# martin-velas/SLAM_plus_plus

Measured on AMD Instinct MI355X. Metric: Lambda solve GFLOP/s (algorithmic factor+solve flops / wall-clock), 100k-pose SE(3), higher is better.
Workload: dtype f64; 1 GPU; C3: synthetic 100000-pose SE(3) chain + loop closures, 6x6 blocks, 201998 upper blocks, n=600000; numeric factor + 2 substitutions per step (symbolic analysis cached, inputs resident in HBM); parallelism=1 GPU

## Files before the change

slam_plus_plus_amd/csrc/preload.h:

```cpp
#pragma once
#include <hip/hip_runtime.h>

#define SLAMPP_PRELOAD_UNIT(unit) \
	namespace slampp { \
	__global__ void preload_##unit##_kernel() {} \
	void preload_##unit(hipStream_t stream) { hipLaunchKernelGGL(preload_##unit##_kernel, dim3(1), dim3(1), 0, stream); } \
	}

namespace slampp {

void preload_simt_kernel(hipStream_t stream);
void preload_panel_kernel(hipStream_t stream);
void preload_sparse_kernels(hipStream_t stream);
void preload_subtree_kernel(hipStream_t stream);
void preload_dense_tiles(hipStream_t stream);
void preload_dense_chol(hipStream_t stream);
void preload_schur(hipStream_t stream);
void preload_schur_tiles(hipStream_t stream);

inline void preload_device_code(hipStream_t stream)
{
	preload_simt_kernel(stream);
	preload_panel_kernel(stream);
	preload_sparse_kernels(stream);
	preload_subtree_kernel(stream);
	preload_dense_tiles(stream);
	preload_dense_chol(stream);
	preload_schur(stream);
	preload_schur_tiles(stream);
}

}
```

slam_plus_plus_amd/csrc/simt_kernel.hip:

```cpp
#include <hip/hip_runtime.h>
#include "sparse_kernels.h"

#include <algorithm>
#include <cstdio>

namespace slampp {

__device__ __forceinline__ double simt_rsqrt(double x)
{
	double y = __builtin_amdgcn_rsq(x);
	const double h = 0.5 * x;
	y = y * (1.5 - h * y * y);
	y = y * (1.5 - h * y * y);
	return y;
}

template <int D>
__device__ __forceinline__ void load_column(const double *__restrict__ p, double (&v)[D])
{
	if(D % 2 == 0) {
		const double2 *p2 = reinterpret_cast<const double2*>(p);
		#pragma unroll
		for(int i = 0; i < D / 2; ++ i) {
			const double2 t = p2[i];
			v[2 * i] = t.x;
			v[2 * i + 1] = t.y;
		}
	} else {
		#pragma unroll
		for(int i = 0; i < D; ++ i)
			v[i] = p[i];
	}
}

template <int D>
__device__ __forceinline__ void load_block(const double *__restrict__ p, double (&v)[D][D])
{
	if(D % 2 == 0) {
		const double2 *p2 = reinterpret_cast<const double2*>(p);
		#pragma unroll
		for(int i = 0; i < D * D / 2; ++ i) {
			const double2 t = p2[i];
			v[(2 * i) / D][(2 * i) % D] = t.x;
			v[(2 * i + 1) / D][(2 * i + 1) % D] = t.y;
		}
	} else {
		#pragma unroll
		for(int i = 0; i < D * D; ++ i)
			v[i / D][i % D] = p[i];
	}
}

template <int D>
__device__ __forceinline__ void load_lower(const double *__restrict__ p, double (&v)[D][D])
{
	#pragma unroll
	for(int q = 0; q < D; ++ q) {
		if(D % 2 == 0) {
			#pragma unroll
			for(int r = q & ~1; r < D; r += 2) {
				const double2 t = *reinterpret_cast<const double2*>(p + r + q * D);
				v[q][r] = t.x;
				v[q][r + 1] = t.y;
			}
		} else {
			#pragma unroll
			for(int r = q; r < D; ++ r)
				v[q][r] = p[r + q * D];
		}
	}
}

template <int D>
__device__ __forceinline__ void store_block(double *p, const double (&m)[D][D])
{
	if(D % 2 == 0) {
		double2 *p2 = reinterpret_cast<double2*>(p);
		#pragma unroll
		for(int q = 0; q < D; ++ q) {
			#pragma unroll
			for(int r = 0; r < D; r += 2)
				p2[(r + q * D) / 2] = double2{m[r][q], m[r + 1][q]};
		}
	} else {
		#pragma unroll
		for(int q = 0; q < D; ++ q) {
			#pragma unroll
			for(int r = 0; r < D; ++ r)
				p[r + q * D] = m[r][q];
		}
	}
}

template <int D>
__device__ __forceinline__ void load_half_rows(const double *__restrict__ p, int r0, double (&v)[D][D / 2])
{
	#pragma unroll
	for(int c = 0; c < D; ++ c) {
		#pragma unroll
		for(int i = 0; i < D / 2; ++ i)
			v[c][i] = p[r0 + i + c * D];
	}
}

__device__ __forceinline__ int pc_next_column(const int32_t *P, int pc, int nb, int nr)
{
	pc += 2 * nr;
	for(int kb = 1; kb < nb; ++ kb)
		pc += 1 + 2 * P[pc];
	return pc;
}

template <int D, int W, int LPT, bool b_linv>
__global__ void __launch_bounds__(64)
factor_simt_kernel(const TSimtChunk *__restrict__ chunks, const int32_t *__restrict__ prog, const long long *__restrict__ tab,
	const double *__restrict__ A, double *L, double *Linv, const double *__restrict__ b, double *w, int *p_flag,
	long long *p_timing, TBatch t_batch)
{	{ const int64_t n_member = blockIdx.y; A += n_member * t_batch.a; L += n_member * t_batch.l; Linv = Linv? Linv + n_member * t_batch.linv : Linv; b += n_member * t_batch.b; w += n_member * t_batch.w; p_flag += n_member; }

	enum { DD = D * D };
	extern __shared__ long long s_tab[];
	const TSimtChunk ch = chunks[blockIdx.x];
	{
		const int n_entries = (4 * prog[ch.prog_off] + prog[ch.prog_off + 1] + prog[ch.prog_off + 2] + prog[ch.prog_off + 3]) * W;
		for(int i = threadIdx.x; i < n_entries; i += 64)
			s_tab[i] = tab[ch.tab_off + i];
		__syncthreads();
	}
	if(int(threadIdx.x) >= W * LPT)
		return;
	const int n_half = (LPT == 2)? int(threadIdx.x) & 1 : 0;
	enum { DH = (LPT == 2)? D / 2 : D };
	const int r0 = n_half * DH;
	long long *p_tm = 0;
	int n_tm = 0;
	if(p_timing && blockIdx.x == gridDim.x / 2 && threadIdx.x == 0) {
		const unsigned long long n_tm_record = atomicAdd((unsigned long long*)p_timing, 1ull);
		p_tm = (n_tm_record < 4096)? p_timing + 1 + 32 * n_tm_record : 0;
		if(p_tm)
			p_tm[n_tm ++] = wall_clock64();
	}
#define SIMT_TICK() do { if(p_tm && n_tm < 32) p_tm[n_tm ++] = wall_clock64(); } while(0)
	const int32_t *P = prog + ch.prog_off;
	const long long *T = s_tab + threadIdx.x / LPT;
// ... 187 lines not shown
				}
			}
			double *p_out = L + l_base + kb * DD;
			#pragma unroll
			for(int q = 0; q < D; ++ q) {
				double out[DH];
				#pragma unroll
				for(int i = 0; i < DH; ++ i) {
					double sum = 0;
					#pragma unroll
					for(int t = 0; t <= q; ++ t)
						sum += acc[i][t] * x[q][t];
					out[i] = sum;
				}
				if(DH % 2 == 0 && D % 2 == 0) {
					#pragma unroll
					for(int i = 0; i < DH; i += 2)
						*reinterpret_cast<double2*>(p_out + r0 + i + q * D) = double2{out[i], out[i + 1]};
				} else {
					#pragma unroll
					for(int i = 0; i < DH; ++ i)
						p_out[r0 + i + q * D] = out[i];
				}
			}
			SIMT_TICK();
		}
		blk0 += nb;
	}
	if(b_bad || f_touched == 1.2345e301)
		atomicOr(p_flag, 1);
}

bool launch_factor_simt(const TSimtChunk *chunks, int n_chunks, int n_width, int n_lds_bytes, const int32_t *prog, const int64_t *tab, int n_dim,
	const double *A, double *L, double *Linv, const double *b, double *w, int *p_flag, hipStream_t stream, long long *p_timing, const TBatch &t_batch)
{
	if(n_chunks <= 0)
		return true;
	const long long *t = reinterpret_cast<const long long*>(tab);
#define SIMT_LAUNCH(D_, W_, LPT_) do { if(Linv) hipLaunchKernelGGL((factor_simt_kernel<D_, W_, LPT_, true>), dim3(n_chunks, t_batch.n), dim3(64), n_lds_bytes, stream, chunks, prog, t, \
	A, L, Linv, b, w, p_flag, p_timing, t_batch); else hipLaunchKernelGGL((factor_simt_kernel<D_, W_, LPT_, false>), dim3(n_chunks, t_batch.n), dim3(64), n_lds_bytes, stream, chunks, prog, t, \
	A, L, Linv, b, w, p_flag, p_timing, t_batch); } while(0)
#define SIMT_WIDTHS(D_) do { if(n_width == 16) { if(b_pairs && D_ % 2 == 0) SIMT_LAUNCH(D_, 16, (D_ % 2 == 0)? 2 : 1); else SIMT_LAUNCH(D_, 16, 1); } \
	else if(n_width == 32) { if(b_pairs && D_ % 2 == 0) SIMT_LAUNCH(D_, 32, (D_ % 2 == 0)? 2 : 1); else SIMT_LAUNCH(D_, 32, 1); } \
	else SIMT_LAUNCH(D_, 64, 1); } while(0)
	const int n_pairs_env = dev_knob("SLAMPP_HIP_DEV_SIMT_PAIRS", -1);
	const bool b_pairs = (n_pairs_env >= 0)? n_pairs_env != 0 : n_chunks <= 2048;
	switch(n_dim) {
	case 3:
		SIMT_WIDTHS(3);
		return true;
	case 6:
		SIMT_WIDTHS(6);
		return true;
	case 7:
		SIMT_WIDTHS(7);
		return true;
	default:
		return false;
	}
#undef SIMT_WIDTHS
#undef SIMT_LAUNCH
}

template <int D, int W>
__global__ void __launch_bounds__(64)
backward_simt_kernel(const TSimtChunk *__restrict__ chunks, const int32_t *__restrict__ prog, const long long *__restrict__ tab,
	const double *__restrict__ L, double *w, double *x_out, TBatch t_batch)
{	{ const int64_t n_member = blockIdx.y; L += n_member * t_batch.l; w += n_member * t_batch.w; x_out += n_member * t_batch.b; }

	enum { DD = D * D };
	extern __shared__ long long s_tab[];
	const TSimtChunk ch = chunks[blockIdx.x];
	const int32_t *P = prog + ch.prog_off;
	const int n_cols = P[0], n_below = P[1];
	{
		const int n_entries = (3 * n_cols + n_below) * W;
		for(int i = threadIdx.x; i < n_entries; i += 64)
			s_tab[i] = tab[ch.tab_off + i];
		__syncthreads();
// ... 421 lines not shown
```

slam_plus_plus_amd/csrc/solver.h:

```cpp
#pragma once
#include <hip/hip_runtime.h>
#include <chrono>
#include <cstdint>
#include <new>
#include <stdexcept>
#include <string>
#include <vector>
#include <thread>
#include <memory>
#include <mutex>

#include "../../include/slampp_hip.h"
#include "plan.h"
#include "host_pool.h"
#include "sparse_records.h"
#include <utility>
#include "sparse_kernels.h"
#include "dense_chol.h"

namespace slampp {

struct CDeviceError : public std::runtime_error {
	explicit CDeviceError(const std::string &s) :std::runtime_error(s) {}
};
// ... 122 lines not shown
	void Refine_Structure();
	bool b_schur_fallback = false;
	int n_staging_ahead = 0;
	int n_schur_fallback_option = 1;
	slampp::Plan plan;
	slampp::SparseLaunchLists lists;
	slampp::TDevPlan dplan;
	slampp::CDevArray<slampp::TColDesc> d_cols;
	slampp::CDevArray<slampp::TBlkDesc> d_blks;
	slampp::CDevArray<slampp::TRowEnt> d_rents;
	slampp::CDevArray<longlong2> d_pairs;
	slampp::CDevArray<int64_t> d_task_ptr, d_task_pkg;
	slampp::CDevArray<longlong2> d_pkg;
	slampp::CDevArray<long long> d_timing;
	slampp::CDevArray<slampp::TSimtChunk> d_simt_chunks;
	slampp::CDevArray<int32_t> d_simt_prog, d_simt_rest;
	int n_panel = -1;
	int n_panel_rows = -1;
	slampp::CDevArray<longlong2> d_panel_pkg;
	slampp::CDevArray<int64_t> d_panel_off, d_panel_out_off;
	slampp::CDevArray<double> d_handup;
	int n_panel_handup = 1;
	slampp::CDevArray<int32_t> d_panel_rest;
	int n_panel_backward = -1;
	size_t n_lds_limit = 0;
	slampp::CDevArray<longlong2> d_bwd_rec;
	slampp::CDevArray<int64_t> d_bwd_off;
	slampp::CDevArray<slampp::TUpdSlot> d_panel_upd_slots;
	slampp::CDevArray<slampp::TUpdEnt> d_panel_upd_ents;
	slampp::CDevArray<int64_t> d_simt_tab;
	slampp::CDevArray<slampp::TSimtChunk> d_simt_bwd_chunks;
	slampp::CDevArray<int32_t> d_simt_bwd_prog;
	slampp::CDevArray<int64_t> d_simt_bwd_tab;
	std::vector<int32_t> simt_bwd_ahead_waves;
	bool b_leaf_linv_wanted = false, b_leaf_linv_valid = true;
	slampp::TBatch t_batch = slampp::t_No_Batch();
	slampp::CDevArray<double> d_batch_L, d_batch_Linv, d_batch_w, d_batch_handup;
	slampp::CDevArray<int> d_batch_flag;
	int n_batch_owner_member = -1;
	int *p_host_batch_flag = 0;
	int n_batch_pending = 0;
	int n_simt_backward = -1;
	void Ensure_Leaf_Inverses();
	int n_simt = -1;
	int n_wide_min_tasks = 8192;
	int n_simt_width = 32;
	int n_simt_stages = 1;
	void Upload_Simt(const slampp::SparseRecords &r_rec);
	void Report_Simt_Backward(const slampp::SparseRecords &r_rec) const;
	slampp::CDevArray<slampp::TDenseBlk> d_dense_blks;
	slampp::CDevArray<int64_t> d_dense_blk_loff;
	slampp::CDevArray<double> d_dense, d_dense_invdiag, d_dense_z, d_dense_x;
	slampp::CDevArray<int32_t> d_dense_gaps;
	int n_dense_gaps;
	slampp::CDevArray<uint8_t> d_dense_unit;
	slampp::CDevArray<longlong2> d_dense_dst;
	slampp::CTileSchedule dense_tiles;
	bool b_dense_tiles;
	bool b_dense_clean;
	int n_dense_top_tiles;
	int n_dense_blks, n_dense_cols, n_dense_dim, n_dense_pad;
	slampp::CDevArray<double> d_A, d_rhs, d_L, d_Linv, d_w, d_cov;
	slampp::CSparseInverse *p_sinv = 0;
	bool b_sinv_tried = false;
	slampp::CCovariance *p_cov = 0;
	slampp::CDevArray<double> d_Z;
	slampp::CDevArray<double> d_Zd, d_Zd_work;
	slampp::CDevArray<int64_t> d_diag_zoff;
	slampp::CDevArray<int32_t> d_diag_dim;
	slampp::CDevArray<int64_t> d_diag_out_off;
	slampp::CDevArray<int64_t> d_damp_off;
	bool b_damp_valid = false;
	bool Require_Damping_Offsets();
	slampp::CDevArray<double> d_lm_reduce;
	slampp::CDevArray<int64_t> d_state_cumsum;
	bool b_state_cumsum_valid = false;
	slampp::CDevArray<int> d_flag;
	int *p_flag_shared = 0;
	int *p_host_flag;

	double *p_pin_values = 0, *p_pin_rhs = 0;
	size_t n_pin_values = 0, n_pin_rhs = 0;
// ... 128 lines not shown
```

slam_plus_plus_amd/csrc/sparse_enqueue.hip:

```cpp
#include <execinfo.h>
#include <signal.h>
#include <unistd.h>
#include <pthread.h>
#include "solver.h"
#include "sparse_inverse.h"

#include <algorithm>
#include <atomic>
#include <chrono>
#include <cstdio>
#include <cstdlib>
#include <cstring>
#include <map>
#include <thread>
#include <mutex>
#include <condition_variable>
#include <functional>
#include <sys/mman.h>

using namespace slampp;

void slampp_hip_solver::Enqueue_Sparse(const double *p_values_dev, double *p_rhs_dev, bool b_factor, bool b_factor_only)
{
	const Plan &P = plan;
// ... 20 lines not shown
		b_panel_fused = b_panel_fused || lists.b_any_hand_up;
		auto Launch_Panels = [&](int s, bool b_bottom) {
			const int n_panels = lists.panel_ptr[s + 1] - lists.panel_ptr[s];
			const bool b_rode = lists.panel_ride[s] != 0;
			if(!b_rode)
				launch_panel_update(P.max_dim, d_panel_upd_slots.p() + lists.panel_upd_ptr[s], lists.panel_upd_ptr[s + 1] - lists.panel_upd_ptr[s],
					d_panel_upd_ents.p(), p_values_dev, d_L.p(), p_rhs_dev, d_w.p(), stream, t_batch);
			const int n_next = (s + 1 < n_stages && lists.panel_ride[s + 1] == 1)? lists.panel_upd_ptr[s + 2] - lists.panel_upd_ptr[s + 1] : 0;
			if(!launch_factor_panel(P.max_dim, b_panel_fused, (n_panel_rows < 0)? P.max_dim >= 6 : n_panel_rows != 0, lists.panel_cfg[s], d_panel_pkg.p(), d_panel_off.p() + lists.panel_ptr[s],
				d_panel_out_off.p() + lists.panel_ptr[s], n_panels,
				d_panel_upd_slots.p() + ((n_next > 0)? lists.panel_upd_ptr[s + 1] : 0), n_next, d_panel_upd_ents.p(), p_values_dev, p_rhs_dev,
				d_L.p(), d_Linv.p(), d_w.p(), d_handup.p(), p_flag, stream, dplan.p_timing, t_batch))
				throw CDeviceError("panel launch refused: block size or LDS request outside what the analysis planned for");
			if(lists.panel_rest_ptr[s + 1] > lists.panel_rest_ptr[s]) {
				TDevPlan t_rest = dplan;
				t_rest.task_map = d_panel_rest.p();
				launch_factor_stage(t_rest, p_values_dev, d_L.p(), d_Linv.p(), p_rhs_dev, d_w.p(), lists.panel_rest_ptr[s],
					lists.panel_rest_ptr[s + 1] - lists.panel_rest_ptr[s], b_bottom, p_flag, stream, t_batch);
			}
		};
		for(int s = 0; s < n_stages; ++ s) {
			if(s == 0)
				Phase_Begin("factor_leaves");
			else if(s == 1 && (b_profile >= 2 || n_wide_end <= 1))
				Phase_Begin((s < n_wide_end)? "factor_wide" : "factor_upper");
			else if(s == 1)
				Phase_Begin("factor_rest");
			else if(s == n_wide_end && b_profile >= 2)
				Phase_Begin("factor_upper");
			if(b_simt && s + 1 < int(lists.simt_chunk_ptr.size())) {
				const int n_chunks = lists.simt_chunk_ptr[s + 1] - lists.simt_chunk_ptr[s], n_rest = lists.simt_rest_ptr[s + 1] - lists.simt_rest_ptr[s];
				const bool b_store_linv = b_leaf_linv_wanted || !b_simt_backward_wanted;
				launch_factor_simt(d_simt_chunks.p() + lists.simt_chunk_ptr[s], n_chunks, n_simt_width, lists.simt_lds_bytes[s], d_simt_prog.p(), d_simt_tab.p(), P.max_dim,
					p_values_dev, d_L.p(), b_store_linv? d_Linv.p() : 0, p_rhs_dev, d_w.p(), p_flag, stream, dplan.p_timing, t_batch);
				b_leaf_linv_valid = b_leaf_linv_valid && b_store_linv;
				if(n_rest > 0) {
					TDevPlan t_rest = dplan;
					t_rest.task_map = d_simt_rest.p();
					launch_factor_stage(t_rest, p_values_dev, d_L.p(), d_Linv.p(), p_rhs_dev, d_w.p(), lists.simt_rest_ptr[s], n_rest,
						true, p_flag, stream, t_batch);
				}
			} else if(s == 0 && !lists.panel_ptr.empty() && lists.panel_ptr[1] > lists.panel_ptr[0]) {
				Launch_Panels(s, true);
			} else if(s > 0 && s < lists.n_bottom_stages && dplan.task_pkg)
				launch_factor_wide(dplan, p_values_dev, d_L.p(), d_Linv.p(), p_rhs_dev, d_w.p(), P.stage_ptr[s],
					P.stage_ptr[s + 1] - P.stage_ptr[s], p_flag, stream, t_batch);
			else if(s >= lists.n_bottom_stages && !lists.panel_ptr.empty()) {
				Launch_Panels(s, false);
			} else
			launch_factor_stage(dplan, p_values_dev, d_L.p(), d_Linv.p(), p_rhs_dev, d_w.p(), P.stage_ptr[s],
				P.stage_ptr[s + 1] - P.stage_ptr[s], s < lists.n_bottom_stages, p_flag, stream, t_batch);
			if(s == 0 || (s == n_wide_end - 1 && b_profile >= 2) || s == n_stages - 1)
				Phase_End();
		}
	} else {
		Phase_Begin("forward");
		for(int s = 0; s < n_stages; ++ s) {
			launch_forward_stage(dplan, d_L.p(), d_Linv.p(), p_rhs_dev, d_w.p(), P.stage_ptr[s],
				P.stage_ptr[s + 1] - P.stage_ptr[s], stream);
		}
		Phase_End();
	}
	if(b_factor_only && !n_dense_dim) {
		SLAMPP_HIP_CHECK(hipGetLastError());
		return;
	}
	if(n_dense_dim) {
// ... 81 lines not shown
```

slam_plus_plus_amd/csrc/sparse_kernels.h:

```cpp
#pragma once
#include <hip/hip_runtime.h>
#include <stdint.h>
#include "plan.h"

namespace slampp {

struct TBatch {
	int n;
	int64_t a, l, linv, b, w, h;
};
inline TBatch t_No_Batch() { TBatch t = {1, 0, 0, 0, 0, 0, 0}; return t; }



struct TColDesc {
	int64_t k0;
	int32_t nb, dj;
	int64_t linv_off;
	int64_t cs_new;
	int64_t cs_src;
	int64_t r0;
	int32_t nr;
	int32_t np;
	int64_t p0;
// ... 140 lines not shown

enum { UP_CHUNK = 16, UP_NR = 128, UP_NP = 512, WIDE_CHUNK = 8, WIDE_NR = 32, WIDE_NP = 48 };
enum { PKG_SPECULATIVE = 512 };

inline __host__ __device__ int package_units(int nb, int ne)
{
	return 4 + 2 * nb + ne + (ne + 3) / 4 + (ne + 15) / 16;
}

struct TDevPlan {
	const TColDesc *cols;
	const TBlkDesc *blks;
	const longlong2 *pairs;
	const TRowEnt *rents;
	const int64_t *task_ptr;
	int uniform_dim;
	int64_t n_blks, n_pairs, n_rents;
	const longlong2 *pkg;
	const int64_t *task_pkg;
	const int32_t *task_map;
	long long *p_timing;
};

struct TSimtChunk {
	int32_t prog_off;
	int32_t n_tasks;
	int64_t tab_off;
};

bool launch_factor_simt(const TSimtChunk *chunks, int n_chunks, int n_width ,
	int n_lds_bytes ,
	const int32_t *prog, const int64_t *tab, int n_dim,
	const double *A, double *L, double *Linv , const double *b, double *w, int *p_flag, hipStream_t stream,
	long long *p_timing = 0 , const TBatch &t_batch = t_No_Batch());
enum { SIMT_BWD_AHEAD = 2 };
bool launch_backward_simt(const TSimtChunk *chunks, int n_chunks, int n_width, int n_lds_bytes, size_t n_lds_limit ,
	int n_ahead_waves, const int32_t *prog, const int64_t *tab,
	int n_dim, const double *L, double *w, double *x_out, hipStream_t stream, const TBatch &t_batch = t_No_Batch(), bool b_report = false);
int backward_simt_ahead_waves(int n_dim, int n_width, int n_lds_bytes);
bool launch_invert_diagonals(const TDevPlan &p, int64_t col_begin, int64_t col_end, const double *L, double *Linv, hipStream_t stream);

void launch_factor_stage(const TDevPlan &p, const double *A, double *L, double *Linv, const double *b,
	double *w, int task_begin, int n_tasks, bool b_bottom_stage, int *p_flag, hipStream_t stream, const TBatch &t_batch = t_No_Batch());
bool launch_factor_subtree_image(const TDevPlan &p, const double *A, double *L, double *Linv, const double *b,
	double *w, int task_begin, int n_tasks, int *p_flag, hipStream_t stream, const TBatch &t_batch = t_No_Batch());
void launch_factor_wide(const TDevPlan &p, const double *A, double *L, double *Linv, const double *b,
	double *w, int task_begin, int n_tasks, int *p_flag, hipStream_t stream, const TBatch &t_batch = t_No_Batch());
void launch_forward_stage(const TDevPlan &p, const double *L, const double *Linv, const double *b,
	double *w, int task_begin, int n_tasks, hipStream_t stream);
void launch_backward_stage(const TDevPlan &p, const double *L, const double *Linv, double *w,
	double *x_out, int task_begin, int n_tasks, hipStream_t stream, const TBatch &t_batch = t_No_Batch());

void launch_dense_assemble(const TDevPlan &p, const TDenseBlk *blks, int n_blks, const double *A, const double *L,
	const double *b, const double *w, double *Dm, int ld, bool b_rhs_only, hipStream_t stream);
void launch_dense_gather_factor(const TDenseBlk *blks, const int64_t *loffs, int n_blks, const double *Dm, int ld, double *L, hipStream_t stream);
void launch_gather_values(const int64_t *p_map, int64_t n, const double *p_src, double *p_dst, hipStream_t stream);

}
```

slam_plus_plus_amd/csrc/sparse_setup.hip:

```cpp
#include <execinfo.h>
#include <signal.h>
#include <unistd.h>
#include <pthread.h>
#include "solver.h"
#include "sparse_inverse.h"
#include "sparse_records.h"

#include <algorithm>
#include <atomic>
#include <chrono>
#include <cstdio>
#include <cstdlib>
#include <cstring>
#include <map>
#include <string>
#include <unordered_map>
#include <thread>
#include <mutex>
#include <condition_variable>
#include <functional>
#include <sys/mman.h>

using namespace slampp;

// ... 344 lines not shown
		for(int32_t c = lists.simt_chunk_ptr[s]; c < lists.simt_chunk_ptr[s + 1]; ++ c) {
			const TSimtChunk &ch = r_rec.simt_bwd_chunks[size_t(c)];
			const int32_t *P = &r_rec.simt_bwd_prog[size_t(ch.prog_off)];
			const int n_cols = P[0], n_below = P[1];
			n_tasks += ch.n_tasks;
			n_spare_chunks += ch.n_tasks < n_simt_width;
			n_by_cols[std::min(n_cols, int(N_MAX))] += ch.n_tasks;
			for(int i = 0, n_blk0 = 0; i < n_cols; n_blk0 += P[2 + i] - 1, ++ i) {
				n_by_blocks[std::min(P[2 + i] - 1, int(N_MAX))] += ch.n_tasks;
				int n_set_outside = 0;
				for(int k = 0; k < SIMT_BWD_AHEAD && k < P[2 + i] - 1; ++ k)
					n_set_outside += P[2 + n_cols + n_blk0 + k] < 0;
				n_by_outside[n_set_outside] += ch.n_tasks;
			}
			for(int b = 0; b < n_below; ++ b)
				((P[2 + n_cols + b] >= 0)? n_inside : n_outside) += ch.n_tasks;
		}
		std::string s_cols, s_blocks, s_outside;
		for(int i = 0; i <= SIMT_BWD_AHEAD; ++ i)
			s_outside += " " + std::to_string(i) + ":" + std::to_string(n_by_outside[i]);
		for(int i = 0; i <= N_MAX; ++ i) {
			if(n_by_cols[i])
				s_cols += " " + std::to_string(i) + ":" + std::to_string(n_by_cols[i]);
			if(n_by_blocks[i])
				s_blocks += " " + std::to_string(i) + ":" + std::to_string(n_by_blocks[i]);
		}
		fprintf(stderr, "[setup] stage %zu backward lanes: %lld tasks in %d chunks of width %d, %d chunks with spare lanes, fetch ahead holds %d blocks, one round holds %d waves; "
			"tasks by columns:%s; columns by sub-diagonal blocks:%s; columns by rows outside the task among the blocks held:%s; blocks with the row inside the task: %lld, outside: %lld\n", s, n_tasks,
			lists.simt_chunk_ptr[s + 1] - lists.simt_chunk_ptr[s], n_simt_width, n_spare_chunks, int(SIMT_BWD_AHEAD),
			(s < simt_bwd_ahead_waves.size())? simt_bwd_ahead_waves[s] : 0, s_cols.c_str(), s_blocks.c_str(), s_outside.c_str(), n_inside, n_outside);
	}
}

void slampp_hip_solver::Upload_Simt(const SparseRecords &r_rec)
{
	const Plan &P = plan;
	if(r_rec.simt_chunks.empty())
		return;
	d_simt_chunks.Upload(r_rec.simt_chunks, stream);
	d_simt_prog.Upload(r_rec.simt_prog, stream);
	d_simt_tab.Upload(r_rec.simt_tab, stream);
	d_simt_rest.Upload(r_rec.simt_rest, stream);
	d_simt_bwd_chunks.Upload(r_rec.simt_bwd_chunks, stream);
	d_simt_bwd_prog.Upload(r_rec.simt_bwd_prog, stream);
	d_simt_bwd_tab.Upload(r_rec.simt_bwd_tab, stream);
	SLAMPP_HIP_CHECK(hipStreamSynchronize(stream));
	simt_bwd_ahead_waves.clear();
	for(size_t s = 0; s < lists.simt_bwd_lds_bytes.size(); ++ s)
		simt_bwd_ahead_waves.push_back(backward_simt_ahead_waves(P.max_dim, n_simt_width, lists.simt_bwd_lds_bytes[s]));
	if(getenv("SLAMPP_HIP_PLAN_TIMING")) {
		Report_Simt_Backward(r_rec);
		for(size_t s = 0; s + 1 < lists.simt_chunk_ptr.size(); ++ s) {
			fprintf(stderr, "[setup] stage %zu: %d tasks -> %d chunks of 64 lanes, %d tasks left to the wave-per-task kernel\n", s,
				P.stage_ptr[s + 1] - P.stage_ptr[s], lists.simt_chunk_ptr[s + 1] - lists.simt_chunk_ptr[s], lists.simt_rest_ptr[s + 1] - lists.simt_rest_ptr[s]);
		}
	}
}
```

Baseline: 570.2 GFLOP/s.

## Add fetch-ahead SIMT factor kernel prefetching next column's Lambda blocks into AGPRs

Adds a new lane-pair SIMT factor kernel for 6x6 blocks. While the current column is being factored, it prefetches the next column's diagonal block, right-hand side and first few sub-diagonal source blocks from Lambda into registers pinned as AGPRs, with manual waitcnt control. The aim is to hide global-load latency behind the Cholesky arithmetic. The kernel is chosen only when the chunk count fits within one occupancy round, and the extra register pressure may lower occupancy.

```diff
diff --git a/slam_plus_plus_amd/csrc/preload.h b/slam_plus_plus_amd/csrc/preload.h
--- a/slam_plus_plus_amd/csrc/preload.h
+++ b/slam_plus_plus_amd/csrc/preload.h
@@ -10,6 +10,7 @@
 namespace slampp {
 
 void preload_simt_kernel(hipStream_t stream);
+void preload_simt_factor_ahead(hipStream_t stream);
 void preload_panel_kernel(hipStream_t stream);
 void preload_sparse_kernels(hipStream_t stream);
 void preload_subtree_kernel(hipStream_t stream);
@@ -21,6 +22,7 @@
 inline void preload_device_code(hipStream_t stream)
 {
 	preload_simt_kernel(stream);
+	preload_simt_factor_ahead(stream);
 	preload_panel_kernel(stream);
 	preload_sparse_kernels(stream);
 	preload_subtree_kernel(stream);
diff --git a/slam_plus_plus_amd/csrc/simt_factor_ahead.hip b/slam_plus_plus_amd/csrc/simt_factor_ahead.hip
--- /dev/null
+++ b/slam_plus_plus_amd/csrc/simt_factor_ahead.hip
@@ -0,0 +1,411 @@
+#include <hip/hip_runtime.h>
+#include "sparse_kernels.h"
+
+#include <algorithm>
+
+namespace slampp {
+
+#include "simt_device.inl"
+
+template <int D, int AHEAD>
+struct TFactorAheadSet {
+	double d[D][D];
+	double b[D];
+	double c[AHEAD][D / 2][D];
+};
+
+template <int D, int AHEAD>
+constexpr int factor_ahead_fetch_loads()
+{
+	int n = D / 2;
+	for(int r = 0; r < D; ++ r)
+		n += r / 2 + 1;
+	return n + AHEAD * (D / 2) * D;
+}
+template <int D> constexpr int factor_ahead_half_block_stores() { return D * ((D / 2) / 2 + (D / 2) % 2); }
+template <int D> constexpr int factor_ahead_diagonal_stores() { return D / 2 + (D / 2) * (D / 2); }
+template <int D> constexpr int factor_ahead_newer_stores() { return (factor_ahead_half_block_stores<D>() < factor_ahead_diagonal_stores<D>())? factor_ahead_half_block_stores<D>() : factor_ahead_diagonal_stores<D>(); }
+constexpr int factor_ahead_wait_imm(int n) { return ((n > 63)? 63 : n) % 16 | 7 << 4 | 15 << 8 | ((n > 63)? 63 : n) / 16 << 14; }
+
+template <int D, int AHEAD>
+__device__ __forceinline__ void factor_ahead_pin(TFactorAheadSet<D, AHEAD> &s)
+{
+	#pragma unroll
+	for(int r = 0; r < D; ++ r) {
+		#pragma unroll
+		for(int q = 0; q < 2 * (r / 2 + 1); ++ q)
+			asm volatile("" : "+a"(s.d[r][q]));
+		asm volatile("" : "+a"(s.b[r]));
+	}
+	#pragma unroll
+	for(int k = 0; k < AHEAD; ++ k) {
+		#pragma unroll
+		for(int i = 0; i < D / 2; ++ i) {
+			#pragma unroll
+			for(int q = 0; q < D; ++ q)
+				asm volatile("" : "+a"(s.c[k][i][q]));
+		}
+	}
+}
+
+template <int D, int W, int AHEAD>
+__device__ __forceinline__ void factor_ahead_fetch(TFactorAheadSet<D, AHEAD> &s, int ci, int n_blk, int nb, int f_blk, int r0, const long long *T,
+	const double *__restrict__ A, const double *__restrict__ b)
+{
+	{
+		const long long enc = T[W * (f_blk + n_blk)];
+		long long n_off = (enc < 0)? 0 : (enc >> 1);
+		asm volatile("" : "+v"(n_off));
+		const double *src = A + n_off;
+		#pragma unroll
+		for(int r = 0; r < D; ++ r) {
+			#pragma unroll
+			for(int i = 0; i <= r / 2; ++ i) {
+				const double2 t = *reinterpret_cast<const double2*>(src + r * D + 2 * i);
+				s.d[r][2 * i] = t.x;
+				s.d[r][2 * i + 1] = t.y;
+			}
+		}
+		load_column<D>(b + T[W * (4 * ci + 3)], s.b);
+	}
+	#pragma unroll
+	for(int k = 0; k < AHEAD; ++ k) {
+		const bool b_exists = k + 1 < nb;
+		const long long enc = T[W * (f_blk + n_blk + (b_exists? k + 1 : 0))];
+		const bool b_trans = b_exists && enc >= 0 && (enc & 1) != 0;
+		long long n_off = (b_exists && enc >= 0)? (enc >> 1) : 0;
+		int n_row_stride = b_trans? D : 1, n_col_stride = b_trans? 1 : D;
+		asm volatile("" : "+v"(n_off), "+v"(n_row_stride), "+v"(n_col_stride));
+		const double *src = A + n_off + r0 * n_row_stride;
+		#pragma unroll
+		for(int i = 0; i < D / 2; ++ i) {
+			#pragma unroll
+			for(int q = 0; q < D; ++ q)
+				s.c[k][i][q] = src[i * n_row_stride + q * n_col_stride];
+		}
+	}
+	asm volatile("" ::: "memory");
+}
+
+template <int D>
+__device__ __forceinline__ void store_half_columns(double *p, const double (&m)[D][D], int n_half)
+{
+	double *p_out = p + n_half * (D / 2) * D;
+	#pragma unroll
+	for(int q = 0; q < D / 2; ++ q) {
+		#pragma unroll
+		for(int r = 0; r < D; r += 2)
+			*reinterpret_cast<double2*>(p_out + r + q * D) = double2{n_half? m[r][q + D / 2] : m[r][q], n_half? m[r + 1][q + D / 2] : m[r + 1][q]};
+	}
+}
+
+template <int D, int W>
+__device__ __forceinline__ void factor_ahead_block(double (&acc)[D / 2][D], const double (&x)[D][D], int &pc, int f_op, int r0, const int32_t *P,
+	const long long *T, double *L, double *p_out)
+{
+	enum { DH = D / 2 };
+	const int np = P[pc ++];
+	{
+		long long off_a = 0, off_b = 0;
+		if(np > 0) {
+			off_a = T[W * (f_op + P[pc])];
+			off_b = T[W * (f_op + P[pc + 1])];
+		}
+		for(int e = 0; e < np; ++ e) {
+			pc += 2;
+			double ca[D][DH], cb[D][D];
+			load_half_rows<D>(L + off_a, r0, ca);
+			load_block<D>(L + off_b, cb);
+			if(e + 1 < np) {
+				off_a = T[W * (f_op + P[pc])];
+				off_b = T[W * (f_op + P[pc + 1])];
+			}
+			#pragma unroll
+			for(int t = 0; t < D; ++ t) {
+				#pragma unroll
+				for(int i = 0; i < DH; ++ i) {
+					#pragma unroll
+					for(int q = 0; q < D; ++ q)
+						acc[i][q] -= ca[t][i] * cb[t][q];
+				}
+			}
+		}
+	}
+	#pragma unroll
+	for(int q = 0; q < D; ++ q) {
+		double out[DH];
+		#pragma unroll
+		for(int i = 0; i < DH; ++ i) {
+			double sum = 0;
+			#pragma unroll
+			for(int t = 0; t <= q; ++ t)
+				sum += acc[i][t] * x[q][t];
+			out[i] = sum;
+		}
+		if(DH % 2 == 0) {
+			#pragma unroll
+			for(int i = 0; i < DH; i += 2)
+				*reinterpret_cast<double2*>(p_out + r0 + i + q * D) = double2{out[i], out[i + 1]};
+		} else {
+			#pragma unroll
+			for(int i = 0; i < DH; ++ i)
+				p_out[r0 + i + q * D] = out[i];
+		}
+	}
+}
+
+template <int D, int W, int LPT, bool b_linv, int AHEAD>
+__global__ void __launch_bounds__(64)
+factor_simt_kernel_ahead(const TSimtChunk *__restrict__ chunks, const int32_t *__restrict__ prog, const long long *__restrict__ tab,
+	const double *__restrict__ A, double *L, double *Linv, const double *__restrict__ b, double *w, int *p_flag,
+	long long *p_timing, TBatch t_batch)
+{	{ const int64_t n_member = blockIdx.y; A += n_member * t_batch.a; L += n_member * t_batch.l; Linv = Linv? Linv + n_member * t_batch.linv : Linv; b += n_member * t_batch.b; w += n_member * t_batch.w; p_flag += n_member; }
+
+	static_assert(LPT == 2 && D % 2 == 0 && AHEAD >= 1, "two lanes per task, even block sizes");
+	enum { DD = D * D, DH = D / 2 };
+	extern __shared__ long long s_tab[];
+	const TSimtChunk ch = chunks[blockIdx.x];
+	{
+		const int n_entries = (4 * prog[ch.prog_off] + prog[ch.prog_off + 1] + prog[ch.prog_off + 2] + prog[ch.prog_off + 3]) * W;
+		for(int i = threadIdx.x; i < n_entries; i += 64)
+			s_tab[i] = tab[ch.tab_off + i];
+		__syncthreads();
+	}
+	if(int(threadIdx.x) >= W * LPT)
+		return;
+	const int n_half = int(threadIdx.x) & 1;
+	const int r0 = n_half * DH;
+	long long *p_tm = 0;
+	int n_tm = 0;
+	if(p_timing && blockIdx.x == gridDim.x / 2 && threadIdx.x == 0) {
+		const unsigned long long n_tm_record = atomicAdd((unsigned long long*)p_timing, 1ull);
+		p_tm = (n_tm_record < 4096)? p_timing + 1 + 32 * n_tm_record : 0;
+		if(p_tm)
+			p_tm[n_tm ++] = wall_clock64();
+	}
+#define SIMT_TICK() do { if(p_tm && n_tm < 32) p_tm[n_tm ++] = wall_clock64(); } while(0)
+	const int32_t *P = prog + ch.prog_off;
+	const long long *T = s_tab + threadIdx.x / LPT;
+	const int n_cols = P[0], n_blocks = P[1], n_ops = P[2];
+	const int f_blk = 4 * n_cols, f_op = f_blk + n_blocks, f_y = f_op + n_ops;
+	int pc = 4, blk0 = 0;
+	bool b_bad = false;
+	TFactorAheadSet<D, AHEAD> t_set;
+	factor_ahead_fetch<D, W, AHEAD>(t_set, 0, 0, P[pc], f_blk, r0, T, A, b);
+	__builtin_amdgcn_s_waitcnt(factor_ahead_wait_imm(0));
+	factor_ahead_pin<D, AHEAD>(t_set);
+	for(int ci = 0; ci < n_cols; ++ ci) {
+		const int nb = P[pc], nr = P[pc + 1], n_touch = P[pc + 2];
+		pc += 3;
+		pc += n_touch;
+		const long long l_base = T[W * (4 * ci)], linv_off = T[W * (4 * ci + 1)], cs_new = T[W * (4 * ci + 2)];
+		__builtin_amdgcn_s_waitcnt(factor_ahead_wait_imm(factor_ahead_newer_stores<D>()));
+		factor_ahead_pin<D, AHEAD>(t_set);
+		double a[D][D], y[D], acc[AHEAD][DH][D];
+		{
+			const long long enc = T[W * (f_blk + blk0)];
+			#pragma unroll
+			for(int r = 0; r < D; ++ r) {
+				#pragma unroll
+				for(int q = 0; q < D; ++ q)
+					a[r][q] = (q <= r && enc >= 0)? t_set.d[r][q] : 0.0;
+			}
+			#pragma unroll
+			for(int r = 0; r < D; ++ r)
+				y[r] = t_set.b[r];
+			#pragma unroll
+			for(int k = 0; k < AHEAD; ++ k) {
+				const bool b_have = k + 1 < nb && T[W * (f_blk + blk0 + ((k + 1 < nb)? k + 1 : 0))] >= 0;
+				#pragma unroll
+				for(int i = 0; i < DH; ++ i) {
+					#pragma unroll
+					for(int q = 0; q < D; ++ q)
+						acc[k][i][q] = b_have? t_set.c[k][i][q] : 0.0;
+				}
+			}
+		}
+		{
+			long long off = 0, yoff = 0;
+			if(nr > 0) {
+				off = T[W * (f_op + P[pc])];
+				yoff = T[W * (f_y + P[pc + 1])];
+			}
+			for(int e = 0; e < nr; ++ e) {
+				pc += 2;
+				double c[D][D], yc[D];
+				load_block<D>(L + off, c);
+				load_column<D>(w + yoff, yc);
+				if(e + 1 < nr) {
+					off = T[W * (f_op + P[pc])];
+					yoff = T[W * (f_y + P[pc + 1])];
+				}
+				#pragma unroll
+				for(int t = 0; t < D; ++ t) {
+					#pragma unroll
+					for(int r = 0; r < D; ++ r) {
+						#pragma unroll
+						for(int q = 0; q <= r; ++ q)
+							a[r][q] -= c[t][r] * c[t][q];
+						y[r] -= c[t][r] * yc[t];
+					}
+				}
+			}
+		}
+		SIMT_TICK();
+		if(ci + 1 < n_cols) {
+			asm volatile("" ::: "memory");
+			factor_ahead_fetch<D, W, AHEAD>(t_set, ci + 1, blk0 + nb, P[pc_next_column(P, pc, nb, 0)], f_blk, r0, T, A, b);
+		}
+		double rd[D];
+		#pragma unroll
+		for(int k = 0; k < D; ++ k) {
+			double piv = a[k][k];
+			const bool b_neg = !(piv > 0);
+			b_bad = b_bad || b_neg;
+			piv = b_neg? 1.0 : piv;
+			const double s = simt_rsqrt(piv);
+			rd[k] = s;
+			a[k][k] = piv * s;
+			#pragma unroll
+			for(int r = k + 1; r < D; ++ r)
+				a[r][k] *= s;
+			#pragma unroll
+			for(int q = k + 1; q < D; ++ q) {
+				#pragma unroll
+				for(int r = q; r < D; ++ r)
+					a[r][q] -= a[r][k] * a[q][k];
+			}
+		}
+		double x[D][D];
+		#pragma unroll
+		for(int c = 0; c < D; ++ c) {
+			#pragma unroll
+			for(int r = 0; r < D; ++ r) {
+				if(r < c)
+					x[r][c] = 0.0;
+				else if(r == c)
+					x[r][c] = rd[r];
+				else {
+					double sum = 0;
+					#pragma unroll
+					for(int t = c; t < r; ++ t)
+						sum += a[r][t] * x[t][c];
+					x[r][c] = -sum * rd[r];
+				}
+			}
+		}
+		{
+			double yn[D];
+			#pragma unroll
+			for(int r = 0; r < D; ++ r) {
+				double sum = 0;
+				#pragma unroll
+				for(int t = 0; t <= r; ++ t)
+					sum += x[r][t] * y[t];
+				yn[r] = sum;
+			}
+			#pragma unroll
+			for(int r = 0; r < D; ++ r) {
+				#pragma unroll
+				for(int q = r + 1; q < D; ++ q)
+					a[r][q] = 0.0;
+			}
+			#pragma unroll
+			for(int r = 0; r < D; r += 2)
+				*reinterpret_cast<double2*>(w + cs_new + r) = double2{yn[r], yn[r + 1]};
+			store_half_columns<D>(L + l_base, a, n_half);
+			if constexpr(b_linv)
+				store_half_columns<D>(Linv + linv_off, x, n_half);
+		}
+		SIMT_TICK();
+		#pragma unroll
+		for(int k = 0; k < AHEAD; ++ k) {
+			if(k + 1 < nb) {
+				factor_ahead_block<D, W>(acc[k], x, pc, f_op, r0, P, T, L, L + l_base + (k + 1) * DD);
+				SIMT_TICK();
+			}
+		}
+		for(int kb = AHEAD + 1; kb < nb; ++ kb) {
+			const long long enc = T[W * (f_blk + blk0 + kb)];
+			double acc_more[DH][D];
+			{
+				const double *src = A + ((enc < 0)? 0 : (enc >> 1));
+				const bool b_trans = (enc & 1) != 0, b_have = enc >= 0;
+				#pragma unroll
+				for(int i = 0; i < DH; ++ i) {
+					#pragma unroll
+					for(int q = 0; q < D; ++ q) {
+						const double f = src[b_trans? q + (r0 + i) * D : (r0 + i) + q * D];
+						acc_more[i][q] = b_have? f : 0.0;
+					}
+				}
+			}
+			factor_ahead_block<D, W>(acc_more, x, pc, f_op, r0, P, T, L, L + l_base + kb * DD);
+			SIMT_TICK();
+		}
+		blk0 += nb;
+	}
+#undef SIMT_TICK
+	if(b_bad)
+		atomicOr(p_flag, 1);
+}
+
+template <int W>
+static const void *p_Factor_Ahead_Kernel(bool b_store_linv)
+{
+	return b_store_linv? reinterpret_cast<const void*>(&factor_simt_kernel_ahead<6, W, 2, true, SIMT_FACTOR_AHEAD>) :
+		reinterpret_cast<const void*>(&factor_simt_kernel_ahead<6, W, 2, false, SIMT_FACTOR_AHEAD>);
+}
+
+static const void *p_Factor_Ahead_Kernel(int n_dim, int n_width, bool b_store_linv)
+{
+	if(n_dim != 6)
+		return 0;
+	return (n_width == 16)? p_Factor_Ahead_Kernel<16>(b_store_linv) : (n_width == 32)? p_Factor_Ahead_Kernel<32>(b_store_linv) : 0;
+}
+
+bool factor_simt_ahead_exists(int n_dim, int n_width)
+{
+	return p_Factor_Ahead_Kernel(n_dim, n_width, false) != 0;
+}
+
+int factor_simt_ahead_waves(int n_dim, int n_width, int n_lds_bytes)
+{
+	int n_device = 0, n_cus = 0, n_waves = 0;
+	if(!factor_simt_ahead_exists(n_dim, n_width) || n_lds_bytes < 0 || hipGetDevice(&n_device) != hipSuccess ||
+	   hipDeviceGetAttribute(&n_cus, hipDeviceAttributeMultiprocessorCount, n_device) != hipSuccess || n_cus <= 0) {
+		(void)hipGetLastError();
+		return 0;
+	}
+	for(int b_store_linv = 0; b_store_linv < 2; ++ b_store_linv) {
+		int n_blocks = 0;
+		if(hipOccupancyMaxActiveBlocksPerMultiprocessor(&n_blocks, p_Factor_Ahead_Kernel(n_dim, n_width, b_store_linv != 0), 64, size_t(n_lds_bytes)) != hipSuccess || n_blocks <= 0) {
+			(void)hipGetLastError();
+			return 0;
+		}
+		n_waves = (b_store_linv)? std::min(n_waves, n_cus * n_blocks) : n_cus * n_blocks;
+	}
+	return n_waves;
+}
+
+bool launch_factor_simt_ahead(const TSimtChunk *chunks, int n_chunks, int n_width, int n_lds_bytes, const int32_t *prog, const int64_t *tab, int n_dim,
+	const double *A, double *L, double *Linv, const double *b, double *w, int *p_flag, hipStream_t stream, long long *p_timing, const TBatch &t_batch)
+{
+	if(!factor_simt_ahead_exists(n_dim, n_width))
+		return false;
+	const long long *t = reinterpret_cast<const long long*>(tab);
+#define AHEAD_LAUNCH(W_, b_linv_) hipLaunchKernelGGL((factor_simt_kernel_ahead<6, W_, 2, b_linv_, SIMT_FACTOR_AHEAD>), dim3(n_chunks, t_batch.n), dim3(64), n_lds_bytes, stream, \
+	chunks, prog, t, A, L, Linv, b, w, p_flag, p_timing, t_batch)
+	if(n_width == 16) {
+		if(Linv) AHEAD_LAUNCH(16, true); else AHEAD_LAUNCH(16, false);
+	} else {
+		if(Linv) AHEAD_LAUNCH(32, true); else AHEAD_LAUNCH(32, false);
+	}
+#undef AHEAD_LAUNCH
+	return true;
+}
+
+}
+
+#include "preload.h"
+SLAMPP_PRELOAD_UNIT(simt_factor_ahead)
diff --git a/slam_plus_plus_amd/csrc/simt_kernel.hip b/slam_plus_plus_amd/csrc/simt_kernel.hip
--- a/slam_plus_plus_amd/csrc/simt_kernel.hip
+++ b/slam_plus_plus_amd/csrc/simt_kernel.hip
@@ -6,110 +6,7 @@
 
 namespace slampp {
 
-__device__ __forceinline__ double simt_rsqrt(double x)
-{
-	double y = __builtin_amdgcn_rsq(x);
-	const double h = 0.5 * x;
-	y = y * (1.5 - h * y * y);
-	y = y * (1.5 - h * y * y);
-	return y;
-}
-
-template <int D>
-__device__ __forceinline__ void load_column(const double *__restrict__ p, double (&v)[D])
-{
-	if(D % 2 == 0) {
-		const double2 *p2 = reinterpret_cast<const double2*>(p);
-		#pragma unroll
-		for(int i = 0; i < D / 2; ++ i) {
-			const double2 t = p2[i];
-			v[2 * i] = t.x;
-			v[2 * i + 1] = t.y;
-		}
-	} else {
-		#pragma unroll
-		for(int i = 0; i < D; ++ i)
-			v[i] = p[i];
-	}
-}
-
-template <int D>
-__device__ __forceinline__ void load_block(const double *__restrict__ p, double (&v)[D][D])
-{
-	if(D % 2 == 0) {
-		const double2 *p2 = reinterpret_cast<const double2*>(p);
-		#pragma unroll
-		for(int i = 0; i < D * D / 2; ++ i) {
-			const double2 t = p2[i];
-			v[(2 * i) / D][(2 * i) % D] = t.x;
-			v[(2 * i + 1) / D][(2 * i + 1) % D] = t.y;
-		}
-	} else {
-		#pragma unroll
-		for(int i = 0; i < D * D; ++ i)
-			v[i / D][i % D] = p[i];
-	}
-}
-
-template <int D>
-__device__ __forceinline__ void load_lower(const double *__restrict__ p, double (&v)[D][D])
-{
-	#pragma unroll
-	for(int q = 0; q < D; ++ q) {
-		if(D % 2 == 0) {
-			#pragma unroll
-			for(int r = q & ~1; r < D; r += 2) {
-				const double2 t = *reinterpret_cast<const double2*>(p + r + q * D);
-				v[q][r] = t.x;
-				v[q][r + 1] = t.y;
-			}
-		} else {
-			#pragma unroll
-			for(int r = q; r < D; ++ r)
-				v[q][r] = p[r + q * D];
-		}
-	}
-}
-
-template <int D>
-__device__ __forceinline__ void store_block(double *p, const double (&m)[D][D])
-{
-	if(D % 2 == 0) {
-		double2 *p2 = reinterpret_cast<double2*>(p);
-		#pragma unroll
-		for(int q = 0; q < D; ++ q) {
-			#pragma unroll
-			for(int r = 0; r < D; r += 2)
-				p2[(r + q * D) / 2] = double2{m[r][q], m[r + 1][q]};
-		}
-	} else {
-		#pragma unroll
-		for(int q = 0; q < D; ++ q) {
-			#pragma unroll
-			for(int r = 0; r < D; ++ r)
-				p[r + q * D] = m[r][q];
-		}
-	}
-}
-
-template <int D>
-__device__ __forceinline__ void load_half_rows(const double *__restrict__ p, int r0, double (&v)[D][D / 2])
-{
-	#pragma unroll
-	for(int c = 0; c < D; ++ c) {
-		#pragma unroll
-		for(int i = 0; i < D / 2; ++ i)
-			v[c][i] = p[r0 + i + c * D];
-	}
-}
-
-__device__ __forceinline__ int pc_next_column(const int32_t *P, int pc, int nb, int nr)
-{
-	pc += 2 * nr;
-	for(int kb = 1; kb < nb; ++ kb)
-		pc += 1 + 2 * P[pc];
-	return pc;
-}
+#include "simt_device.inl"
 
 template <int D, int W, int LPT, bool b_linv>
 __global__ void __launch_bounds__(64)
@@ -363,7 +260,8 @@
 }
 
 bool launch_factor_simt(const TSimtChunk *chunks, int n_chunks, int n_width, int n_lds_bytes, const int32_t *prog, const int64_t *tab, int n_dim,
-	const double *A, double *L, double *Linv, const double *b, double *w, int *p_flag, hipStream_t stream, long long *p_timing, const TBatch &t_batch)
+	const double *A, double *L, double *Linv, const double *b, double *w, int *p_flag, hipStream_t stream, long long *p_timing, const TBatch &t_batch,
+	int n_ahead_waves)
 {
 	if(n_chunks <= 0)
 		return true;
@@ -376,6 +274,15 @@
 	else SIMT_LAUNCH(D_, 64, 1); } while(0)
 	const int n_pairs_env = dev_knob("SLAMPP_HIP_DEV_SIMT_PAIRS", -1);
 	const bool b_pairs = (n_pairs_env >= 0)? n_pairs_env != 0 : n_chunks <= 2048;
+	const int n_ahead_env = dev_knob("SLAMPP_HIP_DEV_SIMT_FACTOR_AHEAD", -1);
+	const int n_lpt = (b_pairs && n_dim % 2 == 0 && (n_width == 16 || n_width == 32))? 2 : 1;
+	const bool b_ahead = n_lpt == 2 && factor_simt_ahead_exists(n_dim, n_width) &&
+		((n_ahead_env >= 0)? n_ahead_env != 0 : int64_t(n_chunks) * std::max<int64_t>(t_batch.n, 1) <= n_ahead_waves);
+	if(p_timing)
+		fprintf(stderr, "stage_timing lane-per-task factor launch: %d chunks, width %d, block size %d, %d members, LPT %d, %s\n", n_chunks, n_width, n_dim,
+			int(t_batch.n), n_lpt, b_ahead? "fetch ahead" : "fetch by column");
+	if(b_ahead)
+		return launch_factor_simt_ahead(chunks, n_chunks, n_width, n_lds_bytes, prog, tab, n_dim, A, L, Linv, b, w, p_flag, stream, p_timing, t_batch);
 	switch(n_dim) {
 	case 3:
 		SIMT_WIDTHS(3);
diff --git a/slam_plus_plus_amd/csrc/solver.h b/slam_plus_plus_amd/csrc/solver.h
--- a/slam_plus_plus_amd/csrc/solver.h
+++ b/slam_plus_plus_amd/csrc/solver.h
@@ -178,6 +178,7 @@
 	slampp::CDevArray<slampp::TSimtChunk> d_simt_bwd_chunks;
 	slampp::CDevArray<int32_t> d_simt_bwd_prog;
 	slampp::CDevArray<int64_t> d_simt_bwd_tab;
+	std::vector<int32_t> simt_factor_ahead_waves;
 	std::vector<int32_t> simt_bwd_ahead_waves;
 	bool b_leaf_linv_wanted = false, b_leaf_linv_valid = true;
 	slampp::TBatch t_batch = slampp::t_No_Batch();
@@ -194,6 +195,7 @@
 	int n_simt_stages = 1;
 	void Upload_Simt(const slampp::SparseRecords &r_rec);
 	void Report_Simt_Backward(const slampp::SparseRecords &r_rec) const;
+	void Report_Simt_Factor(const slampp::SparseRecords &r_rec) const;
 	slampp::CDevArray<slampp::TDenseBlk> d_dense_blks;
 	slampp::CDevArray<int64_t> d_dense_blk_loff;
 	slampp::CDevArray<double> d_dense, d_dense_invdiag, d_dense_z, d_dense_x;
diff --git a/slam_plus_plus_amd/csrc/sparse_enqueue.hip b/slam_plus_plus_amd/csrc/sparse_enqueue.hip
--- a/slam_plus_plus_amd/csrc/sparse_enqueue.hip
+++ b/slam_plus_plus_amd/csrc/sparse_enqueue.hip
@@ -76,7 +76,8 @@
 				const int n_chunks = lists.simt_chunk_ptr[s + 1] - lists.simt_chunk_ptr[s], n_rest = lists.simt_rest_ptr[s + 1] - lists.simt_rest_ptr[s];
 				const bool b_store_linv = b_leaf_linv_wanted || !b_simt_backward_wanted;
 				launch_factor_simt(d_simt_chunks.p() + lists.simt_chunk_ptr[s], n_chunks, n_simt_width, lists.simt_lds_bytes[s], d_simt_prog.p(), d_simt_tab.p(), P.max_dim,
-					p_values_dev, d_L.p(), b_store_linv? d_Linv.p() : 0, p_rhs_dev, d_w.p(), p_flag, stream, dplan.p_timing, t_batch);
+					p_values_dev, d_L.p(), b_store_linv? d_Linv.p() : 0, p_rhs_dev, d_w.p(), p_flag, stream, dplan.p_timing, t_batch,
+					(size_t(s) < simt_factor_ahead_waves.size())? simt_factor_ahead_waves[size_t(s)] : 0);
 				b_leaf_linv_valid = b_leaf_linv_valid && b_store_linv;
 				if(n_rest > 0) {
 					TDevPlan t_rest = dplan;
diff --git a/slam_plus_plus_amd/csrc/sparse_kernels.h b/slam_plus_plus_amd/csrc/sparse_kernels.h
--- a/slam_plus_plus_amd/csrc/sparse_kernels.h
+++ b/slam_plus_plus_amd/csrc/sparse_kernels.h
@@ -196,7 +196,13 @@
 	int n_lds_bytes ,
 	const int32_t *prog, const int64_t *tab, int n_dim,
 	const double *A, double *L, double *Linv , const double *b, double *w, int *p_flag, hipStream_t stream,
-	long long *p_timing = 0 , const TBatch &t_batch = t_No_Batch());
+	long long *p_timing = 0 , const TBatch &t_batch = t_No_Batch(),
+	int n_ahead_waves = 0 );
+enum { SIMT_FACTOR_AHEAD = 2 };
+bool factor_simt_ahead_exists(int n_dim, int n_width);
+bool launch_factor_simt_ahead(const TSimtChunk *chunks, int n_chunks, int n_width, int n_lds_bytes, const int32_t *prog, const int64_t *tab, int n_dim,
+	const double *A, double *L, double *Linv, const double *b, double *w, int *p_flag, hipStream_t stream, long long *p_timing, const TBatch &t_batch);
+int factor_simt_ahead_waves(int n_dim, int n_width, int n_lds_bytes);
 enum { SIMT_BWD_AHEAD = 2 };
 bool launch_backward_simt(const TSimtChunk *chunks, int n_chunks, int n_width, int n_lds_bytes, size_t n_lds_limit ,
 	int n_ahead_waves, const int32_t *prog, const int64_t *tab,
diff --git a/slam_plus_plus_amd/csrc/sparse_setup.hip b/slam_plus_plus_amd/csrc/sparse_setup.hip
--- a/slam_plus_plus_amd/csrc/sparse_setup.hip
+++ b/slam_plus_plus_amd/csrc/sparse_setup.hip
@@ -400,6 +400,58 @@
 	}
 }
 
+void slampp_hip_solver::Report_Simt_Factor(const SparseRecords &r_rec) const
+{
+	enum { N_MAX = 16 };
+	for(size_t s = 0; s + 1 < lists.simt_chunk_ptr.size(); ++ s) {
+		long long n_by_cols[N_MAX + 1] = {0}, n_by_blocks[N_MAX + 1] = {0}, n_by_sources[N_MAX + 1] = {0}, n_by_fill[N_MAX + 1] = {0}, n_held_fill = 0, n_tasks = 0;
+		int n_spare_chunks = 0;
+		for(int32_t c = lists.simt_chunk_ptr[s]; c < lists.simt_chunk_ptr[s + 1]; ++ c) {
+			const TSimtChunk &ch = r_rec.simt_chunks[size_t(c)];
+			const int32_t *P = &r_rec.simt_prog[size_t(ch.prog_off)];
+			const int64_t *T = &r_rec.simt_tab[size_t(ch.tab_off)];
+			const int n_cols = P[0];
+			n_tasks += ch.n_tasks;
+			n_spare_chunks += ch.n_tasks < n_simt_width;
+			n_by_cols[std::min(n_cols, int(N_MAX))] += ch.n_tasks;
+			for(int i = 0, pc = 4, n_blk0 = 0; i < n_cols; ++ i) {
+				const int nb = P[pc], nr = P[pc + 1], n_touch = P[pc + 2];
+				pc += 3 + n_touch + 2 * nr;
+				for(int kb = 1; kb < nb; ++ kb)
+					pc += 1 + 2 * P[pc];
+				n_by_blocks[std::min(nb - 1, int(N_MAX))] += ch.n_tasks;
+				for(int t = 0; t < ch.n_tasks; ++ t) {
+					int n_sources = 0, n_fill = 0;
+					for(int kb = 1; kb < nb; ++ kb) {
+						const bool b_fill = T[size_t(4 * n_cols + n_blk0 + kb) * size_t(n_simt_width) + size_t(t)] < 0;
+						(b_fill? n_fill : n_sources) ++;
+						n_held_fill += b_fill && kb <= int(SIMT_FACTOR_AHEAD);
+					}
+					n_by_sources[std::min(n_sources, int(N_MAX))] ++;
+					n_by_fill[std::min(n_fill, int(N_MAX))] ++;
+				}
+				n_blk0 += nb;
+			}
+		}
+		std::string s_cols, s_blocks, s_sources, s_fill;
+		for(int i = 0; i <= N_MAX; ++ i) {
+			if(n_by_cols[i])
+				s_cols += " " + std::to_string(i) + ":" + std::to_string(n_by_cols[i]);
+			if(n_by_blocks[i])
+				s_blocks += " " + std::to_string(i) + ":" + std::to_string(n_by_blocks[i]);
+			if(n_by_sources[i])
+				s_sources += " " + std::to_string(i) + ":" + std::to_string(n_by_sources[i]);
+			if(n_by_fill[i])
+				s_fill += " " + std::to_string(i) + ":" + std::to_string(n_by_fill[i]);
+		}
+		fprintf(stderr, "[setup] stage %zu factor lanes: %lld tasks in %d chunks of width %d, %d chunks with spare lanes, fetch ahead holds %d blocks, one round holds %d waves; "
+			"tasks by columns:%s; columns by sub-diagonal blocks:%s; columns by sub-diagonal blocks with a source in Lambda:%s; columns by fill-in blocks:%s; "
+			"fill-in blocks among the blocks held: %lld\n", s, n_tasks, lists.simt_chunk_ptr[s + 1] - lists.simt_chunk_ptr[s], n_simt_width, n_spare_chunks,
+			int(SIMT_FACTOR_AHEAD), (s < simt_factor_ahead_waves.size())? simt_factor_ahead_waves[s] : 0, s_cols.c_str(), s_blocks.c_str(), s_sources.c_str(),
+			s_fill.c_str(), n_held_fill);
+	}
+}
+
 void slampp_hip_solver::Upload_Simt(const SparseRecords &r_rec)
 {
 	const Plan &P = plan;
@@ -416,8 +468,12 @@
 	simt_bwd_ahead_waves.clear();
 	for(size_t s = 0; s < lists.simt_bwd_lds_bytes.size(); ++ s)
 		simt_bwd_ahead_waves.push_back(backward_simt_ahead_waves(P.max_dim, n_simt_width, lists.simt_bwd_lds_bytes[s]));
+	simt_factor_ahead_waves.clear();
+	for(size_t s = 0; s < lists.simt_lds_bytes.size(); ++ s)
+		simt_factor_ahead_waves.push_back(factor_simt_ahead_waves(P.max_dim, n_simt_width, lists.simt_lds_bytes[s]));
 	if(getenv("SLAMPP_HIP_PLAN_TIMING")) {
 		Report_Simt_Backward(r_rec);
+		Report_Simt_Factor(r_rec);
 		for(size_t s = 0; s + 1 < lists.simt_chunk_ptr.size(); ++ s) {
 			fprintf(stderr, "[setup] stage %zu: %d tasks -> %d chunks of 64 lanes, %d tasks left to the wave-per-task kernel\n", s,
 				P.stage_ptr[s + 1] - P.stage_ptr[s], lists.simt_chunk_ptr[s + 1] - lists.simt_chunk_ptr[s], lists.simt_rest_ptr[s + 1] - lists.simt_rest_ptr[s]);
```

New measurement: 587.3 GFLOP/s (median of 6 runs). +3.0%, better.
